# tprodanov/locityper

Hardware: AMD Instinct MI355X
Metric: reads/s through the whole genotyping path (scored + prefiltered + default solver scheme); reads_scored_per_s and genotypes_solved_per_s give the two halves (higher is better)
Workload: dtype f64

## Files before the change

### locityper_amd/csrc/lcty_api.hip

```cpp
#include <algorithm>
#include <cmath>
#include <memory>
#include <numeric>

#include "lcty_objects.hpp"

using namespace lcty;

namespace lcty {
static thread_local std::string g_last_error;
thread_local hipStream_t tl_stream = nullptr;
void set_last_error(const std::string& msg) { g_last_error = msg; }
}

hipEvent_t lcty_ctx::get_event() {
    hipEvent_t e;
    if (!event_pool.empty()) { e = event_pool.back(); event_pool.pop_back(); return e; }
    LCTY_HIP(hipEventCreate(&e));
    return e;
}

void lcty_ctx::fold_oldest(lcty::KernelTimer& t, size_t count) {
    count = std::min(count, t.pending.size());
    for (size_t i = 0; i < count; i++) {
        float ms = 0.f;
        LCTY_HIP(hipEventSynchronize(t.pending[i].second));
        LCTY_HIP(hipEventElapsedTime(&ms, t.pending[i].first, t.pending[i].second));
        t.total_ms += ms; t.launches++;
        event_pool.push_back(t.pending[i].first); event_pool.push_back(t.pending[i].second);
    }
    t.pending.erase(t.pending.begin(), t.pending.begin() + static_cast<std::ptrdiff_t>(count));
}

extern "C" {

int32_t lcty_ctx_set_knob(lcty_ctx* ctx, const char* name, int64_t value) {
    return guarded([&] {
        if (!ctx || !name) fail(LCTY_ERR_INVALID_INPUT, "null argument");
        static const char* const known[] = {"transfer_levels", "transfer_scratch_mb", "transfer_waves", "transfer_cap_new", "transfer_arena",
                                            "depth_table_start", "solve_budget_mb", "solve_chains_per_wave", "solve_extra_start", "solve_lds_weights",
                                            "anneal_lds_weights", "contig_info_slide", "gather_chunk_mb", "prefilter_gram", "prefilter_gram_cols",
                                            "prefilter_gram_levels", "comm_fail_at", "score_lean", "arena_cap_pct", "exact_threads", "host_threads",
                                            "score_lean_keep", "score_lean_two", "queue_early_head", "db_chunk_cols", "basis_batch_words",
                                            "align_batch_pairs", "align_hash_bits", "align_dp_cells", "align_match_budget", "align_cigar_store_mb", "pafvcf_hash_bits", "pafvcf_table_mb",
                                            "genome_max_bases", "sample_bam_hash_bits", "sample_bam_max_slice_bytes", "sample_bam_inflate",
                                            "bgzf_deflate", "bgzf_deflate_max_bytes", "aln_bam_max_slice_bytes", "vcf_max_slice_bytes",
#ifdef LCTY_DIAG
                                            "solve_stats", "queue_trace", "map_trace", "exact_trace", "solve_greedy_form", "solve_anneal_timing", "score_timing",
                                            "solve_init_tiles", "transfer_phases", "genome_scan_form",
#endif
                                            nullptr};
        bool ok = false;
        for (const char* const* k = known; *k; k++) ok |= strcmp(*k, name) == 0;
        if (!ok) fail(LCTY_ERR_INVALID_INPUT, "unknown knob '%s'", name);
        if (strcmp(name, "bgzf_deflate") == 0 && value != 0 && value != 1) fail(LCTY_ERR_INVALID_INPUT, "bgzf_deflate = %lld (0: host, 1: device)", static_cast<long long>(value));
        if (value < 0) ctx->knobs.erase(name); else ctx->knobs[name] = value;
    });
}

int32_t lcty_ctx_set_path(lcty_ctx* ctx, const char* name, const char* path) {
    return guarded([&] {
        if (!ctx || !name) fail(LCTY_ERR_INVALID_INPUT, "null argument");
        if (strcmp(name, "exact_dump") != 0) fail(LCTY_ERR_INVALID_INPUT, "unknown path '%s'", name);
        ctx->exact_dump_path = path ? path : "";
    });
}

const char* lcty_last_error(void) { return g_last_error.c_str(); }
const char* lcty_version(void) { return "locityper_hip 0.1.0 (gfx950)"; }

int32_t lcty_device_count(void) {
    int n = 0;
    if (hipGetDeviceCount(&n) != hipSuccess) { (void)hipGetLastError(); return 0; }
    return n;
}

int32_t lcty_ctx_create(int32_t device_id, lcty_ctx** out) {
    return guarded([&] {
        if (!out) fail(LCTY_ERR_INVALID_INPUT, "null argument");
        int n = 0;
        if (hipGetDeviceCount(&n) != hipSuccess || n == 0) {
            (void)hipGetLastError();
            fail(LCTY_ERR_RUNTIME, "no HIP device is visible: liblocityper_hip has no CPU fallback");
        }
        if (device_id < 0 || device_id >= n) fail(LCTY_ERR_INVALID_INPUT, "device %d out of range (0..%d)", device_id, n - 1);
        auto c = std::unique_ptr<lcty_ctx>(new lcty_ctx());
        c->device = device_id;
        LCTY_HIP(hipSetDevice(device_id));
        LCTY_HIP(hipGetDeviceProperties(&c->props, device_id));
        LCTY_HIP(hipStreamCreateWithFlags(&c->stream.main, hipStreamNonBlocking));
        *out = c.release();
    });
}
// ... 322 lines not shown
```

### locityper_amd/csrc/lcty_solve_device.hpp

```cpp
#pragma once
#include "lcty_objects.hpp"

namespace lcty {

constexpr uint32_t MAXP = 4;
constexpr uint32_t NONE32S = 0xFFFFFFFFu;
constexpr uint32_t MID_NONE24 = 0xFFFFFFu;
constexpr uint64_t WINDOW_KEY_XOR = 0xD1B54A32D192ED03ull;
constexpr uint64_t INIT_KEY_XOR = 0x8CB92BA72F3D8DD7ull;

struct FastDiv {
    uint32_t d, m, s1, s2;
    __host__ static FastDiv make(uint32_t d) {
        FastDiv f{d, 0, 0, 0};
        uint32_t l = 0;
        while ((1ull << l) < d) l++;
        f.m = static_cast<uint32_t>(((1ull << 32) * ((1ull << l) - d)) / d + 1);
        f.s1 = l < 1 ? l : 1; f.s2 = l > 0 ? l - 1 : 0;
        return f;
    }
    __device__ __forceinline__ uint32_t div(uint32_t n) const {
        const uint32_t t = __umulhi(m, n);
        return (t + ((n - t) >> s1)) >> s2;
    }
// ... 58 lines not shown
    uint32_t* c_uc;
    uint8_t* c_gc;
    uint32_t* c_depth;
    uint32_t* c_nnt;
    double* c_aln;
    double* liks;
    double* parts;
    uint32_t* overflow;
    double* dbg;
    uint32_t edge_trivial;
};

__device__ __forceinline__ uint64_t uniform64(uint64_t x) {
    const uint32_t lo = __builtin_amdgcn_readfirstlane(static_cast<uint32_t>(x));
    const uint32_t hi = __builtin_amdgcn_readfirstlane(static_cast<uint32_t>(x >> 32));
    return (static_cast<uint64_t>(hi) << 32) | lo;
}
__device__ __forceinline__ uint64_t counter_u64(uint64_t key, uint64_t i) {
    uint64_t z = key + (i + 1) * 0x9e3779b97f4a7c15ull;
    z = (z ^ (z >> 30)) * 0xbf58476d1ce4e5b9ull;
    z = (z ^ (z >> 27)) * 0x94d049bb133111ebull;
    return z ^ (z >> 31);
}
struct Xoshiro {
    uint64_t s0, s1, s2, s3;
    __device__ __forceinline__ void seed(uint64_t x) {
        s0 = counter_u64(x, 0); s1 = counter_u64(x, 1); s2 = counter_u64(x, 2); s3 = counter_u64(x, 3);
    }
    __device__ __forceinline__ uint64_t next() {
        const uint64_t sum = s0 + s3;
        const uint64_t result = ((sum << 23) | (sum >> 41)) + s0;
        const uint64_t t = s1 << 17;
        s2 ^= s0; s3 ^= s1; s1 ^= s2; s0 ^= s3; s2 ^= t; s3 = (s3 << 45) | (s3 >> 19);
        return result;
    }
    __device__ __forceinline__ uint64_t below(uint64_t n) { return __umul64hi(next(), n); }
    __device__ __forceinline__ double f64() { return static_cast<double>(next() >> 11) * (1.0 / 9007199254740992.0); }
};

constexpr uint32_t INIT_SEGS = 4;
struct RecList {
    ChainRec* base; const uint32_t* cum; uint32_t seg_reads;
    uint32_t r1 = 0, r2 = 0, r3 = 0; bool in_regs = false;
    __device__ __forceinline__ uint32_t place(uint32_t s) const {
        const uint32_t c1 = in_regs ? r1 : cum[1], c2 = in_regs ? r2 : cum[2], c3 = in_regs ? r3 : cum[3];
        const uint32_t k = (s >= c1 ? 1u : 0u) + (s >= c2 ? 1u : 0u) + (s >= c3 ? 1u : 0u);
        const uint32_t before = s >= c3 ? c3 : s >= c2 ? c2 : s >= c1 ? c1 : 0u;
        return s - before + k * seg_reads;
    }
    __device__ __forceinline__ ChainRec& operator[](uint32_t s) const { return base[place(s)]; }
};

constexpr uint32_t INIT_TILE_T = 8, INIT_TILE_R = 6;
constexpr uint32_t INIT_TILE_Q = 1024;
static_assert(INIT_TILE_Q >= 64 * (INIT_TILE_T + 1) && (INIT_TILE_Q & (INIT_TILE_Q - 1)) == 0, "the list holds a block's entries");
struct __attribute__((aligned(16))) InitChainP {
    uint64_t seed;
    uint32_t chain;
    uint32_t ia, ib;
    uint32_t row0, row1;
    uint32_t id0, id1;
    uint32_t shift0, rs0, re0, shift1, rs1, re1;
    uint32_t total_w;
};
static_assert(sizeof(InitChainP) == 64, "InitChainP layout");
struct __attribute__((aligned(16))) InitGroup { uint32_t first, n_chains, n_rows, _pad; uint32_t row[8]; };
static_assert(sizeof(InitGroup) == 48 && INIT_TILE_R <= 8, "InitGroup layout");
struct InitPlan {
    std::vector<InitGroup> groups; std::vector<InitChainP> chains;
    uint32_t T = 0, R = 0;
    size_t lds = 0;
};

inline void set_rec_list(SolveView& V, uint64_t n_reads) {
    V.seg_reads = static_cast<uint32_t>(((n_reads + INIT_SEGS - 1) / INIT_SEGS + 63) / 64 * 64);
    if (V.seg_reads == 0) V.seg_reads = 64;
    V.rstride = static_cast<uint64_t>(INIT_SEGS) * V.seg_reads;
}
inline size_t init_chain_lds(uint32_t wstride) { return ((static_cast<size_t>(wstride) * 4 + 15) & ~static_cast<size_t>(15)) + 256 * 8 + 64; }

template <typename... P, typename... A>
void launch_lds(lcty_ctx* ctx, int timer, void (*kernel)(P...), dim3 grid, dim3 block, size_t lds, hipStream_t s, const A&... args) {
    if (lds > 48 * 1024)
        LCTY_HIP(hipFuncSetAttribute(reinterpret_cast<const void*>(kernel), hipFuncAttributeMaxDynamicSharedMemorySize, static_cast<int>(lds)));
    auto go = [&] { hipLaunchKernelGGL(kernel, grid, block, lds, s, args...); };
    if (timer < 0) go();
    else ctx->timed(timer, go, s);
    LCTY_HIP(hipGetLastError());
}

void check_solver(const lcty_solver* solver);

void ensure_solver_tables(lcty_reads* reads);
void ensure_depth_table(lcty_locus* loc, uint64_t want);
void build_depth_table_into(const lcty_locus* loc, uint32_t depth, DevBuf<double>& out, hipStream_t s);
bool solver_lds_fits(uint32_t wstride);
struct InitHost {
    const uint16_t* genotypes; const uint64_t* seeds; const uint16_t* row_of; const lcty_locus* loc; uint32_t n_cus;
    uint32_t lds_budget;
};
void plan_init_groups(const SolveView& V, const InitHost& H, uint32_t nch, InitPlan& plan);
void launch_init(lcty_ctx* ctx, const SolveView& V, uint32_t nch, size_t lds_init, hipStream_t s, const InitHost* host, lcty_ctx::SolveWorkspace& ws,
                 InitPlan& plan);
void launch_greedy_chains(lcty_ctx* ctx, SolveView& V, uint32_t nch, hipStream_t stream, lcty_ctx::SolveWorkspace& ws);
void launch_anneal(lcty_ctx* ctx, const SolveView& V, uint32_t nch, hipStream_t s);
void launch_pause(hipStream_t s);
void launch_store_cur(ChainRec* recs, const uint32_t* words, uint64_t n, hipStream_t s);
void launch_pack_rows_count(uint64_t n, const LocCell* table, uint64_t ngp, uint32_t n_good, const uint16_t* alleles, uint32_t n_rows,
                            unsigned long long* total, hipStream_t s);
void launch_pack_rows(uint64_t n, const LocCell* table, const uint32_t* table_ext, const double* table_unm, uint64_t ngp, uint32_t n_good,
                      const uint16_t* alleles, uint32_t n_rows, const PairAlnDev* pa, LocEntry* cells, uint64_t out_stride, PairAlnDev* extras,
                      unsigned long long* cursor, hipStream_t s);
void launch_place_rows(uint64_t n, const LocEntry* cells, uint64_t in_stride, uint32_t n_good, uint32_t n_rows, uint32_t ext_base, LocCell* full,
                       uint32_t* full_ext, double* full_unm, bool write_unm, uint64_t full_stride, uint64_t first, hipStream_t s);
void launch_pad_rows(uint64_t n, LocCell* full, uint32_t* full_ext, double* full_unm, uint64_t full_stride, uint64_t from, uint32_t n_rows, hipStream_t s);
void launch_count_unexplained(uint32_t blocks, const uint8_t* status, const double* unmapped, const double* matrix, uint64_t n_pairs, uint32_t A,
                              const uint16_t* ids, uint32_t ploidy, unsigned long long* out, hipStream_t s);
void launch_read_nw(const SolveView& V, uint32_t* nw, hipStream_t s);
void launch_assignment_counts(const SolveView& V, const uint32_t* nw, const uint64_t* read_off, uint16_t* counts, hipStream_t s);

}
```

### locityper_amd/csrc/lcty_solve_kernels.hip

```cpp
#include <algorithm>
#include <cmath>
#include <type_traits>
#include <vector>

#include "lcty_solve_device.hpp"

namespace lcty {


__global__ __launch_bounds__(256) void build_loc_table_kernel(const uint32_t* __restrict__ good_ix, uint32_t n_good, uint64_t ngp,
                                                              uint32_t A, const uint32_t* __restrict__ pa_idx,
                                                              const uint64_t* __restrict__ pa_off, const PairAlnDev* __restrict__ pa,
                                                              const double* __restrict__ unmapped, LocCell* __restrict__ table,
                                                              uint32_t* __restrict__ table_ext, double* __restrict__ table_unm,
                                                              uint32_t* __restrict__ err) {
    __shared__ LocCell tile[32][33];
    __shared__ uint32_t tile_ext[32][33];
    const uint32_t g0 = blockIdx.x * 32, c0 = blockIdx.y * 32;
    const uint32_t tx = threadIdx.x & 31u, ty = threadIdx.x >> 5;
    if (blockIdx.y == 0 && threadIdx.x < 32) {
        const uint32_t g = g0 + threadIdx.x;
        if (g < ngp) table_unm[g] = g < n_good ? unmapped[good_ix[g]] : 0.0;
    }
    for (uint32_t i = ty; i < 32; i += 8) {
// ... 368 lines not shown
            LocIter<P> it; it.start(L);
            LocOut o;
            for (uint32_t t = 0; t < min(L.nw, 255u) && it.next(L, V, o); t++) {
                uint32_t wa, wb;
                loc_windows(V, G, o, seed, rp, t, &wa, &wb);
                const uint32_t win = wa | (wb << 16);
                if (t == 0) { rec.lp0 = o.lp; rec.win0 = win; }
                else if (t == 1) { rec.lp1 = o.lp; rec.win1 = win; }
                else if (room) { ExtraLoc e; e.lp = o.lp; e.win = win; e._pad = 0; extra[eix + t - 2] = e; }
                if (t == a0) {
                    atomicAdd(&depth[wa], 1u);
                    atomicAdd(&depth[wb], 1u);
                    aln_part += o.lp;
                }
            }
            if (nontrivial) recs[slot] = rec;
        }
    }
    if (lane == 0) seg_cnt[wave] = n_recs;
    red[tid] = aln_part;
    __syncthreads();
    const uint32_t ex_total = seg_cnt[4];
    if (tid == 0) {
        if (ex_total > V.extra_cap) { atomicMax(V.overflow, 4u); atomicMax(V.overflow + 1, ex_total); }
        if (ex_total >= (1u << 24)) atomicMax(V.overflow, 2u);
    }
    for (uint32_t s = 128; s > 0; s >>= 1) {
        if (tid < s) red[tid] += red[tid + s];
        __syncthreads();
    }
    uint32_t* gdepth = V.c_depth + static_cast<uint64_t>(chain) * V.wstride;
    for (uint32_t w = tid; w < G.total_w; w += 256) gdepth[w] = depth[w];
    if (tid == 0) {
        uint32_t* cum = V.c_seg + static_cast<uint64_t>(chain) * 4;
        uint32_t run = 0;
        for (uint32_t k = 0; k < INIT_SEGS; k++) { cum[k] = run; run += seg_cnt[k]; }
        V.c_aln[chain] = red[0]; V.c_nnt[chain] = run; V.c_totw[chain] = G.total_w;
    }
}

__device__ __forceinline__ uint64_t counter_fin(uint64_t z) {
    z = (z ^ (z >> 30)) * 0xbf58476d1ce4e5b9ull;
    z = (z ^ (z >> 27)) * 0x94d049bb133111ebull;
    return z ^ (z >> 31);
}
constexpr uint64_t GOLDEN64 = 0x9e3779b97f4a7c15ull;
typedef uint32_t u32x4_t __attribute__((ext_vector_type(4)));
__device__ __forceinline__ void store_16(uint4* p, uint4 v) {
    u32x4_t x; x.x = v.x; x.y = v.y; x.z = v.z; x.w = v.w;
    __builtin_nontemporal_store(x, reinterpret_cast<u32x4_t*>(p));
}
__host__ __device__ inline size_t init_tile_lds(uint32_t T, uint32_t R, uint32_t wstride) {
    const size_t depth = (static_cast<size_t>(T) * wstride * 4 + 15) & ~static_cast<size_t>(15);
    return depth + static_cast<size_t>(T) * 256 * 8 + 4ull * R * 64 * 16 + static_cast<size_t>(T) * 4 * 8 + static_cast<size_t>(T) * 4 * 5 + 64;
}

__device__ __forceinline__ void init_tile_deferred(const SolveView& V, const InitChainP* __restrict__ cp, uint32_t T, uint32_t* depth, double* aln_def,
                                                   uint32_t* ex_cnt, unsigned long long* queue, uint32_t head, uint32_t n, uint32_t wave, uint32_t lane, bool random_start) {
    double add = 0.0;
    uint32_t my_c = 0xFFFFFFFFu;
    if (lane < n) {
        const unsigned long long packed = __hip_atomic_load(&queue[(head + lane) & (INIT_TILE_Q - 1)], __ATOMIC_RELAXED, __HIP_MEMORY_SCOPE_WORKGROUP);
        const uint2 item = make_uint2(static_cast<uint32_t>(packed), static_cast<uint32_t>(packed >> 32));
        const uint32_t c = item.x >> 24, rp = item.x & 0xFFFFFFu, slot = item.y;
        const InitChainP P = cp[c];
        Geno<2> G;
        G.id[0] = P.id0; G.id[1] = P.id1; G.row[0] = P.row0; G.row[1] = P.row1; G.shift[0] = P.shift0; G.shift[1] = P.shift1;
        G.reg_start[0] = P.rs0; G.reg_start[1] = P.rs1; G.reg_end[0] = P.re0; G.reg_end[1] = P.re1; G.total_w = P.total_w;
        Locs<2> L;
        locs_init<2>(L, V, rp, G);
        if (L.nw > 255) atomicMax(V.overflow, 2u);
        uint32_t a0 = 0;
        if (L.nw > 1 && random_start)
            a0 = static_cast<uint32_t>(__umul64hi(counter_u64(P.seed ^ INIT_KEY_XOR, rp), static_cast<uint64_t>(L.nw)));
        const uint32_t nloc = min(L.nw, 255u), n_extra = nloc > 2 ? nloc - 2u : 0u;
        uint32_t eix = 0;
        if (n_extra) eix = atomicAdd(&ex_cnt[c], n_extra);
        const bool room = static_cast<uint64_t>(eix) + n_extra <= V.extra_cap;
        ExtraLoc* extra = V.extra + static_cast<uint64_t>(P.chain) * V.extra_cap;
        ChainRec rec; rec.rp_cur = rp | (a0 << 24); rec.meta = nloc | (eix << 8);
        rec.lp0 = rec.lp1 = 0.0; rec.win0 = rec.win1 = 0;
        LocIter<2> it; it.start(L);
        LocOut o;
        for (uint32_t t = 0; t < nloc && it.next(L, V, o); t++) {
            uint32_t wa, wb;
            loc_windows(V, G, o, P.seed, rp, t, &wa, &wb);
            const uint32_t win = wa | (wb << 16);
            if (t == 0) { rec.lp0 = o.lp; rec.win0 = win; }
            else if (t == 1) { rec.lp1 = o.lp; rec.win1 = win; }
            else if (room) { ExtraLoc e; e.lp = o.lp; e.win = win; e._pad = 0; extra[eix + t - 2] = e; }
            if (t == a0) {
                atomicAdd(&depth[static_cast<size_t>(c) * V.wstride + wa], 1u);
                atomicAdd(&depth[static_cast<size_t>(c) * V.wstride + wb], 1u);
                add = o.lp;
                my_c = c;
            }
        }
        if (L.nw > 1) V.recs[static_cast<uint64_t>(P.chain) * V.rstride + static_cast<uint64_t>(wave) * V.seg_reads + slot] = rec;
    }
    for (uint32_t c = 0; c < T; c++) {
        unsigned long long m = __ballot(my_c == c);
        if (!m) continue;
        double acc = aln_def[c * 4 + wave];
        while (m) {
            const int l = __ffsll(static_cast<long long>(m)) - 1;
            acc += __hiloint2double(__builtin_amdgcn_readlane(__double2hiint(add), l), __builtin_amdgcn_readlane(__double2loint(add), l));
            m &= m - 1;
        }
        if (lane == 0) aln_def[c * 4 + wave] = acc;
    }
}

__global__ __launch_bounds__(256) void solve_init_tile_kernel(const SolveView V, const InitGroup* __restrict__ groups, const InitChainP* __restrict__ chains,
                                                             unsigned long long* lists, const uint32_t T_max, const uint32_t R_max) {
    extern __shared__ __align__(16) uint8_t smem[];
    const uint32_t tid = threadIdx.x, lane = tid & 63u, wave = __builtin_amdgcn_readfirstlane(tid >> 6);
    const InitGroup& grp = groups[blockIdx.x];
    const uint32_t T = grp.n_chains, R = grp.n_rows;
    const InitChainP* __restrict__ cp = chains + grp.first;
    const uint32_t W = V.wstride;
    uint32_t* depth = reinterpret_cast<uint32_t*>(smem);
    size_t at = (static_cast<size_t>(T_max) * W * 4 + 15) & ~static_cast<size_t>(15);
    double* aln = reinterpret_cast<double*>(smem + at); at += static_cast<size_t>(T_max) * 256 * 8;
    uint4* stage = reinterpret_cast<uint4*>(smem + at) + static_cast<size_t>(wave) * R_max * 64; at += 4ull * R_max * 64 * 16;
    unsigned long long* queue = lists + (static_cast<size_t>(blockIdx.x) * 4 + wave) * INIT_TILE_Q;
    double* aln_def = reinterpret_cast<double*>(smem + at); at += static_cast<size_t>(T_max) * 4 * 8;
    uint32_t* ex_cnt = reinterpret_cast<uint32_t*>(smem + at); at += static_cast<size_t>(T_max) * 4;
    uint32_t* seg_cnt = reinterpret_cast<uint32_t*>(smem + at);

    for (uint32_t c = 0; c < T; c++) {
        const InitChainP P = cp[c];
        double* ww = V.c_ww + static_cast<uint64_t>(P.chain) * W;
        uint8_t* wgc = V.c_gc + static_cast<uint64_t>(P.chain) * W;
        uint32_t* wuc = V.n_wk ? V.c_uc + static_cast<uint64_t>(P.chain) * W : nullptr;
        for (uint32_t w = tid; w < P.total_w; w += 256) {
            depth[c * W + w] = 0;
            double weight = 0.0; uint32_t g = 0, uc = V.n_wk - 1;
            if (w >= 2) {
                const bool second = w >= P.shift1;
                const uint32_t allele = second ? P.id1 : P.id0, sh = second ? P.shift1 : P.shift0, rs = second ? P.rs1 : P.rs0;
                const uint32_t start = rs + (w - sh) * V.window, end = start + V.window;
                const uint32_t left = min(V.tweak, start), right = min(V.tweak, V.allele_len[allele] - end);
                const uint64_t r = counter_u64(P.seed ^ WINDOW_KEY_XOR, w);
                const int64_t off = -static_cast<int64_t>(left) + static_cast<int64_t>(__umul64hi(r, static_cast<uint64_t>(left + right + 1)));
                const uint32_t wstart = static_cast<uint32_t>(static_cast<int64_t>(start) + off);
                const uint32_t i = V.ci_off[allele] + (wstart > V.left_padding ? wstart - V.left_padding : 0u);
                weight = V.win_weight[i];
                g = V.gc[i];
                if (wuc) uc = V.uniq_cnt[i] | (static_cast<uint32_t>(V.compl_cnt[i]) << 16);
                if (weight < V.min_weight || weight < 1e-7) { weight = 0.0; g = 0; uc = V.n_wk - 1; }
            }
            ww[w] = weight; wgc[w] = static_cast<uint8_t>(g);
            if (wuc) wuc[w] = uc;
        }
        aln[c * 256 + tid] = 0.0;
        if (tid < 4) aln_def[c * 4 + tid] = 0.0;
        if (tid == 0) ex_cnt[c] = 0;
    }
    __syncthreads();

    const bool random_start = V.solver.kind == LCTY_SOLVER_ANNEAL || (V.solver.kind == LCTY_SOLVER_GREEDY && !V.solver.best_start);
    const uint32_t seg_lo = min(wave * V.seg_reads, V.n_good), seg_hi = min(seg_lo + V.seg_reads, V.n_good);
    uint64_t row_at[INIT_TILE_R];
#pragma unroll
    for (uint32_t r = 0; r < INIT_TILE_R; r++) row_at[r] = static_cast<uint64_t>(grp.row[r < R ? r : 0]) * V.ngp;
    const uint4* __restrict__ table = reinterpret_cast<const uint4*>(V.table);
    uint4 nxt[INIT_TILE_R]; double nxt_unm = 0.0;
#pragma unroll
    for (uint32_t r = 0; r < INIT_TILE_R; r++) nxt[r] = make_uint4(0, 0, 0, 0);
    if (seg_lo + lane < seg_hi) {
#pragma unroll
        for (uint32_t r = 0; r < INIT_TILE_R; r++) if (r < R) nxt[r] = table[row_at[r] + seg_lo + lane];
        nxt_unm = V.table_unm[seg_lo + lane];
    }
    uint32_t n_recs_all = 0;
    uint32_t qn = 0, qhead = 0;
    for (uint32_t base = seg_lo; base < seg_hi; base += 64) {
        const uint32_t rp = base + lane;
        const bool in = rp < seg_hi;
#pragma unroll
        for (uint32_t r = 0; r < INIT_TILE_R; r++) if (r < R) stage[r * 64 + lane] = nxt[r];
        const double unm = nxt_unm;
        if (rp + 64 < seg_hi) {
#pragma unroll
            for (uint32_t r = 0; r < INIT_TILE_R; r++) if (r < R) nxt[r] = table[row_at[r] + rp + 64];
            nxt_unm = V.table_unm[rp + 64];
        }
        const uint64_t zbase = ((static_cast<uint64_t>(rp) << 16) + 1ull) * GOLDEN64;
        const uint64_t abase = (static_cast<uint64_t>(rp) + 1ull) * GOLDEN64;
        for (uint32_t c = 0; c < T; c++) {
            const InitChainP P = cp[c];
            const uint4 qa = stage[P.ia * 64 + lane], qb = stage[P.ib * 64 + lane];
            const double aln_before = aln[c * 256 + tid];
            const double lpA = __hiloint2double(static_cast<int>(qa.y), static_cast<int>(qa.x));
            const double lpB = __hiloint2double(static_cast<int>(qb.y), static_cast<int>(qb.x));
            const uint32_t rawA = qa.z >> 24, rawB = qb.z >> 24;
            const double thresh = fmax(fmax(lpA, lpB), unm) - V.prob_diff;
            const bool kA = in && rawA != 0 && lpA >= thresh, kB = in && rawB != 0 && lpB >= thresh, kU = in && unm >= thresh;
            const bool multi = (kA && rawA > 1) || (kB && rawB > 1);
            const uint32_t nw = (kA ? 1u : 0u) + (kB ? 1u : 0u) + (kU ? 1u : 0u);
            bool nontrivial = nw > 1;
            if (__any(multi && nw == 1)) {
                if (multi && nw == 1) {
                    const uint32_t ext = V.table_ext[static_cast<uint64_t>(kA ? P.row0 : P.row1) * V.ngp + rp];
                    nontrivial = V.pa[ext].ln_prob >= thresh;
                }
            }
            const unsigned long long nt_mask = __ballot(nontrivial);
            const uint32_t before = __builtin_amdgcn_readlane(n_recs_all, c);
            const uint32_t slot = before + static_cast<uint32_t>(__popcll(nt_mask & ((1ull << lane) - 1ull)));
            {
                const uint32_t after = __builtin_amdgcn_readfirstlane(before + static_cast<uint32_t>(__popcll(nt_mask)));
                uint32_t m0_was;
                asm volatile("s_mov_b32 %1, m0\n\ts_mov_b32 m0, %3\n\tv_writelane_b32 %0, %2, m0\n\ts_mov_b32 m0, %1"
                             : "+v"(n_recs_all), "=&s"(m0_was) : "s"(after), "s"(c));
            }
            const unsigned long long mm = __ballot(multi);
            if (mm) {
                if (multi)
                    __hip_atomic_store(&queue[(qhead + qn + static_cast<uint32_t>(__popcll(mm & ((1ull << lane) - 1ull)))) & (INIT_TILE_Q - 1)],
                                       static_cast<unsigned long long>(rp | (c << 24)) | (static_cast<unsigned long long>(slot) << 32), __ATOMIC_RELAXED,
                                       __HIP_MEMORY_SCOPE_WAVEFRONT);
                qn += static_cast<uint32_t>(__popcll(mm));
            }
            const bool BgtA = lpB > lpA, UgtA = unm > lpA, UgtB = unm > lpB;
            const uint32_t posA = ((kB && BgtA) ? 1u : 0u) + ((kU && UgtA) ? 1u : 0u);
            const uint32_t posB = ((kA && !BgtA) ? 1u : 0u) + ((kU && UgtB) ? 1u : 0u);
            uint32_t tA1 = 0, tA2 = 0, tB1 = 0, tB2 = 0;
            if (V.tweak) {
                const uint64_t z0 = P.seed + zbase;
                const uint64_t rA = counter_fin(z0 + (posA == 0 ? 0ull : posA == 1 ? GOLDEN64 : 2ull * GOLDEN64));
                const uint64_t rB = counter_fin(z0 + (posB == 0 ? 0ull : posB == 1 ? GOLDEN64 : 2ull * GOLDEN64));
                tA1 = V.by_tweak.mod(static_cast<uint32_t>(rA >> 32)); tA2 = V.by_tweak.mod(static_cast<uint32_t>(rA));
                tB1 = V.by_tweak.mod(static_cast<uint32_t>(rB >> 32)); tB2 = V.by_tweak.mod(static_cast<uint32_t>(rB));
            }
            auto window_ix = [&](uint32_t mid, bool none, uint32_t tw, uint32_t rs, uint32_t re, uint32_t sh) -> uint32_t {
                const uint32_t m = mid + tw;
                uint32_t q = V.by_window.div(m - rs) + sh;
                asm volatile("" : "+v"(q));
                const uint32_t inside = (rs <= m && m < re) ? q : 1u;
                return none ? 0u : inside;
            };
            const uint32_t midA1 = qa.z & MID_NONE24, midB1 = qb.z & MID_NONE24;
            const uint32_t winA = window_ix(midA1, midA1 == MID_NONE24, tA1, P.rs0, P.re0, P.shift0) |
                                  (window_ix(qa.w, qa.w == NONE32S, tA2, P.rs0, P.re0, P.shift0) << 16);
            const uint32_t winB = window_ix(midB1, midB1 == MID_NONE24, tB1, P.rs1, P.re1, P.shift1) |
                                  (window_ix(qb.w, qb.w == NONE32S, tB2, P.rs1, P.re1, P.shift1) << 16);
            const bool a_0 = kA && posA == 0, b_0 = kB && posB == 0, a_1 = kA && posA == 1, b_1 = kB && posB == 1, a_2 = kA && posA == 2, b_2 = kB && posB == 2;
            const double lp0 = a_0 ? lpA : (b_0 ? lpB : unm), lp1 = a_1 ? lpA : (b_1 ? lpB : unm), lp2 = a_2 ? lpA : (b_2 ? lpB : unm);
            const uint32_t win0 = a_0 ? winA : (b_0 ? winB : 0u), win1 = a_1 ? winA : (b_1 ? winB : 0u), win2 = a_2 ? winA : (b_2 ? winB : 0u);
            uint32_t a0 = 0;
            double lps = lp0; uint32_t wins = win0;
            if (random_start) {
                const uint64_t r = counter_fin((P.seed ^ INIT_KEY_XOR) + abase);
                a0 = nw > 1 ? static_cast<uint32_t>(__umul64hi(r, static_cast<uint64_t>(nw))) : 0u;
                lps = a0 == 0 ? lp0 : (a0 == 1 ? lp1 : lp2); wins = a0 == 0 ? win0 : (a0 == 1 ? win1 : win2);
            }
            const bool fast = !multi && nw != 0;
            if (fast) {
                atomicAdd(&depth[c * W + (wins & 0xFFFFu)], 1u);
                atomicAdd(&depth[c * W + (wins >> 16)], 1u);
                aln[c * 256 + tid] = aln_before + lps;
            }
            uint32_t eix = 0;
            if (fast && nw == 3) {
                eix = atomicAdd(&ex_cnt[c], 1u);
                if (eix < V.extra_cap) {
                    ExtraLoc e; e.lp = lp2; e.win = win2; e._pad = 0;
                    V.extra[static_cast<uint64_t>(P.chain) * V.extra_cap + eix] = e;
                }
            }
            if (fast && nw > 1) {
                uint4* dst = reinterpret_cast<uint4*>(V.recs + static_cast<uint64_t>(P.chain) * V.rstride + static_cast<uint64_t>(wave) * V.seg_reads + slot);
                store_16(dst, make_uint4(rp | (a0 << 24), nw | (eix << 8), static_cast<uint32_t>(__double2loint(lp0)), static_cast<uint32_t>(__double2hiint(lp0))));
                store_16(dst + 1, make_uint4(static_cast<uint32_t>(__double2loint(lp1)), static_cast<uint32_t>(__double2hiint(lp1)), win0, win1));
            }
        }
        const bool last = base + 64 >= seg_hi;
        if (qn >= 64 || (last && qn)) {
            __builtin_amdgcn_fence(__ATOMIC_RELEASE, "workgroup");
            __builtin_amdgcn_wave_barrier();
            __builtin_amdgcn_fence(__ATOMIC_ACQUIRE, "workgroup");
            while (qn >= 64 || (last && qn)) {
                const uint32_t n = min(qn, 64u);
                init_tile_deferred(V, cp, T, depth, aln_def, ex_cnt, queue, qhead, n, wave, lane, random_start);
                qhead = (qhead + n) & (INIT_TILE_Q - 1); qn -= n;
            }
        }
    }
    if (lane < T) seg_cnt[lane * 4 + wave] = n_recs_all;
    __syncthreads();
    for (uint32_t c = 0; c < T; c++) {
        const InitChainP P = cp[c];
        const uint32_t ex_total = ex_cnt[c];
        if (tid == 0) {
            if (ex_total > V.extra_cap) { atomicMax(V.overflow, 4u); atomicMax(V.overflow + 1, ex_total); }
            if (ex_total >= (1u << 24)) atomicMax(V.overflow, 2u);
        }
        uint32_t* gdepth = V.c_depth + static_cast<uint64_t>(P.chain) * W;
        for (uint32_t w = tid; w < P.total_w; w += 256) gdepth[w] = depth[c * W + w];
        if (wave == 0) {
            double v = (aln[c * 256 + lane] + aln[c * 256 + 64 + lane]) + (aln[c * 256 + 128 + lane] + aln[c * 256 + 192 + lane]);
            for (int o = 32; o > 0; o >>= 1) v += __shfl_xor(v, o);
            v += (aln_def[c * 4] + aln_def[c * 4 + 1]) + (aln_def[c * 4 + 2] + aln_def[c * 4 + 3]);
            if (lane == 0) {
                uint32_t* cum = V.c_seg + static_cast<uint64_t>(P.chain) * 4;
                uint32_t run = 0;
                for (uint32_t k = 0; k < INIT_SEGS; k++) { cum[k] = run; run += seg_cnt[c * 4 + k]; }
                V.c_aln[P.chain] = v; V.c_nnt[P.chain] = run; V.c_totw[P.chain] = P.total_w;
            }
        }
    }
}

struct PairGather { int32_t c[2]; uint32_t dmax[2]; double weight[2], vnew[2], vold[2]; };
__device__ __forceinline__ double pair_term(const PairGather& g, int i, uint32_t* deepest) {
    const bool live = g.c[i] != 0 && g.weight[i] != 0.0;
    *deepest = max(*deepest, live ? g.dmax[i] : 0u);
    return live ? g.weight[i] * g.vnew[i] - g.weight[i] * g.vold[i] : 0.0;
}

__device__ __forceinline__ double lut_at(const double* lut, uint32_t index) {
    return *reinterpret_cast<const double*>(reinterpret_cast<const char*>(lut) + (index << 3));
}
constexpr uint32_t DEPTH_MASK = 0x1FFFFFFu;
struct WinGathered {
    static constexpr bool WEIGHTS_LAST = false;
    uint32_t* wd;
    const double* ww;
    struct Word { uint32_t word; };
    __device__ __forceinline__ Word at(uint32_t w) const { return Word{wd[w]}; }
    __device__ __forceinline__ uint32_t depth(Word x) const { return x.word & DEPTH_MASK; }
    __device__ __forceinline__ uint32_t gc(Word x) const { return x.word >> 25; }
    __device__ __forceinline__ double weight(Word x, uint32_t w) const { return ww[w]; }
};
constexpr uint32_t LW_DEPTH_BITS = 23, LW_DEPTH_MASK = (1u << LW_DEPTH_BITS) - 1u;
struct WinTables {
    static constexpr bool WEIGHTS_LAST = true;
    uint32_t* wd;
    const uint16_t* wh;
    const double* wk; const double* wc;
    struct Word { uint32_t word, half; };
    __device__ __forceinline__ Word at(uint32_t w) const { return Word{wd[w], wh[w]}; }
    __device__ __forceinline__ uint32_t depth(Word x) const { return x.word & LW_DEPTH_MASK; }
    __device__ __forceinline__ uint32_t gc(Word x) const { return x.half & 0x7Fu; }
    __device__ __forceinline__ double weight(Word x, uint32_t w) const { return wk[x.word >> LW_DEPTH_BITS] * wc[x.half >> 7]; }
};

template <typename LAYOUT>
struct Chain {
    const SolveView* V;
    LAYOUT L;
    using Word = typename LAYOUT::Word;
    __device__ __forceinline__ double wlp_at(uint32_t w) const {
        const Word x = L.at(w);
// ... 1041 lines not shown
    int64_t mode = ctx->knob("anneal_lds_weights", tables ? 2 : 0);
    if (mode == 2 && !tables) mode = 0;
    if (mode == 2) launch_anneal_as<2>(ctx, V, nch, s);
    else if (mode == 1) launch_anneal_as<1>(ctx, V, nch, s);
    else launch_anneal_as<0>(ctx, V, nch, s);
}

void launch_greedy_chains(lcty_ctx* ctx, SolveView& V, uint32_t nch, hipStream_t stream, lcty_ctx::SolveWorkspace& ws) {
    const uint32_t S = V.solver.sample_size;
    const uint64_t simds = 4ull * static_cast<uint64_t>(ctx->props.multiProcessorCount);
    uint32_t lpc = S <= 16 ? 16 : S <= 32 ? 32 : 64;
    if (lpc == 16 && (nch + 3) / 4 > simds) {
        if (S <= 12 && (nch + 4) / 5 <= simds) lpc = 12;
        else if (S <= 10) lpc = 10;
        else if (S <= 12) lpc = 12;
    }
    const int64_t want = ctx->knob("solve_chains_per_wave", 0);
    if (want > 0) {
        const uint32_t forced = want >= 6 ? 10u : want == 5 ? 12u : static_cast<uint32_t>(64 / std::min<int64_t>(want, 4));
        if (forced >= S) lpc = forced;
    }
    const bool lw = V.n_wk != 0 && 2 * static_cast<uint64_t>(V.n_good) + 2 <= LW_DEPTH_MASK && ctx->knob("solve_lds_weights", 1) != 0;
    while (lpc < 64 && greedy_lds(lpc, V, lw) > 80 * 1024) lpc = lpc < 16 ? 16 : lpc * 2;
    auto go = [&](auto tag) {
        constexpr uint32_t L = decltype(tag)::value;
        if (lw) launch_greedy<L, true>(ctx, V, nch, stream); else launch_greedy<L, false>(ctx, V, nch, stream);
    };
    const bool timed_form = lpc == 12 && lw && (ctx->diag_knob("solve_greedy_form", 0) & 32) != 0;
    const size_t n_waves = (static_cast<size_t>(nch) + 4) / 5 + 2;
    V.dbg = nullptr;
    if (timed_form) { ws.dbg.ensure(12 * n_waves); ws.dbg.zero(stream); V.dbg = ws.dbg.p; }
    if (lpc == 10) go(std::integral_constant<uint32_t, 10>{});
    else if (lpc == 12) go(std::integral_constant<uint32_t, 12>{});
    else if (lpc == 16) go(std::integral_constant<uint32_t, 16>{});
    else if (lpc == 32) go(std::integral_constant<uint32_t, 32>{});
    else go(std::integral_constant<uint32_t, 64>{});
    if (timed_form) {
        std::vector<double> d(12 * n_waves);
        ws.dbg.download(d.data(), d.size(), stream);
        LCTY_HIP(hipStreamSynchronize(stream));
        double sum[12] = {0}; size_t used = 0;
        for (size_t w = 0; w < n_waves; w++) if (d[12 * w + 6] > 0) { used++; for (int k = 0; k < 12; k++) sum[k] += d[12 * w + k] / d[12 * w + 6]; }
        if (used) fprintf(stderr, "[lcty greedy phases] %zu wavefronts; clock ticks per iteration: candidates+requests %.0f (waiting for the further locations %.0f, current location %.0f, its pair %.0f, first alternative %.0f), ext+sample+record request %.0f, wait+score %.0f, row best %.0f, move %.0f; loop total %.0f; a round for the second alternative in %.3f of the iterations\n",
                          used, sum[0] / used, sum[11] / used, sum[8] / used, sum[9] / used, sum[10] / used, sum[1] / used, sum[2] / used, sum[3] / used, sum[4] / used, sum[5] / used, sum[7] / used);
    }
}

bool solver_lds_fits(uint32_t wstride) {
    return !(static_cast<size_t>(wstride) * 12 + sizeof(AnnealRing) + 128 > 160 * 1024 || wstride > 65535);
}
void plan_init_groups(const SolveView& V, const InitHost& H, uint32_t nch, InitPlan& plan) {
    plan.groups.clear(); plan.chains.clear(); plan.T = plan.R = 0; plan.lds = 0;
    const uint32_t attempts = V.attempts, ng = (nch + attempts - 1) / attempts, A = V.A;
    uint32_t T_cap = INIT_TILE_T;
    const size_t lds_budget = H.lds_budget ? H.lds_budget : 80 * 1024;
    while (T_cap > 1 && init_tile_lds(T_cap, std::min(INIT_TILE_R, T_cap + 1), V.wstride) > lds_budget) T_cap--;
    const uint64_t per_cu = std::max<uint64_t>(1, std::min<uint64_t>(160 * 1024 / init_tile_lds(T_cap, std::min(INIT_TILE_R, T_cap + 1), V.wstride), 4));
    const uint64_t places = per_cu * std::max(1u, H.n_cus);
    T_cap = static_cast<uint32_t>(std::max<uint64_t>(1, std::min<uint64_t>(T_cap, (nch + places - 1) / places)));
    const uint32_t R_cap = std::min(INIT_TILE_R, T_cap + 1);
    std::vector<uint32_t> deg(A, 0), rank(A, 0), order(A);
    for (uint32_t g = 0; g < ng; g++) { deg[H.genotypes[2 * g]]++; deg[H.genotypes[2 * g + 1]]++; }
    for (uint32_t a = 0; a < A; a++) order[a] = a;
    std::stable_sort(order.begin(), order.end(), [&](uint32_t x, uint32_t y) { return deg[x] > deg[y]; });
    for (uint32_t r = 0; r < A; r++) rank[order[r]] = r;
    std::vector<uint32_t> gts(ng);
    std::vector<uint64_t> key(ng);
    for (uint32_t g = 0; g < ng; g++) {
        const uint32_t ra = rank[H.genotypes[2 * g]], rb = rank[H.genotypes[2 * g + 1]];
        const uint64_t u = std::min(ra, rb), v = std::max(ra, rb);
        key[g] = ((u / 2) << 48) | ((v / 4) << 32) | (u << 16) | v;
        gts[g] = g;
    }
    std::sort(gts.begin(), gts.end(), [&](uint32_t x, uint32_t y) { return key[x] != key[y] ? key[x] < key[y] : x < y; });
    auto row_of = [&](uint32_t allele) -> uint32_t { return H.row_of ? H.row_of[allele] : allele; };
    struct Unit { uint32_t gi, a0, n; };
    struct Proto { std::vector<Unit> units; uint32_t n_chains = 0, n_rows = 0; uint32_t row[8] = {0, 0, 0, 0, 0, 0, 0, 0}; };
    std::vector<Proto> protos;
    Proto cur;
    auto close = [&] { if (cur.n_chains) protos.push_back(cur); cur = Proto{}; };
    auto fresh_rows = [&](const Proto& p, uint32_t r0, uint32_t r1) -> uint32_t {
        bool h0 = false, h1 = false;
        for (uint32_t r = 0; r < p.n_rows; r++) { h0 |= p.row[r] == r0; h1 |= p.row[r] == r1; }
        return (h0 ? 0u : 1u) + ((h1 || r1 == r0) ? 0u : 1u);
    };
    auto add_rows = [&](Proto& p, uint32_t r0, uint32_t r1) {
        for (uint32_t x : {r0, r1}) {
            bool have = false;
            for (uint32_t r = 0; r < p.n_rows; r++) have |= p.row[r] == x;
            if (!have) p.row[p.n_rows++] = x;
        }
    };
    for (uint32_t gi : gts) {
        const uint32_t r0 = row_of(H.genotypes[2 * gi]), r1 = row_of(H.genotypes[2 * gi + 1]);
        for (uint32_t a0 = 0; a0 < attempts;) {
            const uint32_t want = std::min(attempts - a0, T_cap);
            if (cur.n_chains + want > T_cap || cur.n_rows + fresh_rows(cur, r0, r1) > R_cap) close();
            add_rows(cur, r0, r1);
            cur.units.push_back(Unit{gi, a0, want}); cur.n_chains += want;
            a0 += want;
        }
    }
    close();
    std::stable_sort(protos.begin(), protos.end(), [](const Proto& a, const Proto& b) { return a.n_chains > b.n_chains; });
    if (protos.size() > places) {
        uint64_t tail_chains = 0;
        for (size_t i = places; i < protos.size(); i++) tail_chains += protos[i].n_chains;
        const uint32_t piece = static_cast<uint32_t>(std::max<uint64_t>(1, std::min<uint64_t>(T_cap, tail_chains / (3 * places))));
        std::vector<Proto> tail;
        for (size_t i = places; i < protos.size(); i++) {
            Proto part;
            for (const Unit& u : protos[i].units)
                for (uint32_t done = 0; done < u.n;) {
                    const uint32_t take = std::min(u.n - done, piece - part.n_chains);
                    add_rows(part, row_of(H.genotypes[2 * u.gi]), row_of(H.genotypes[2 * u.gi + 1]));
                    part.units.push_back(Unit{u.gi, u.a0 + done, take}); part.n_chains += take;
                    done += take;
                    if (part.n_chains == piece) { tail.push_back(part); part = Proto{}; }
                }
            if (part.n_chains) tail.push_back(part);
        }
        protos.resize(places);
        protos.insert(protos.end(), tail.begin(), tail.end());
    }
    for (const Proto& p : protos) {
        InitGroup g{};
        g.first = static_cast<uint32_t>(plan.chains.size()); g.n_rows = p.n_rows;
        for (uint32_t r = 0; r < 8; r++) g.row[r] = p.row[r];
        for (const Unit& u : p.units) {
            const uint32_t id0 = H.genotypes[2 * u.gi], id1 = H.genotypes[2 * u.gi + 1];
            const uint32_t row0 = row_of(id0), row1 = row_of(id1);
            uint32_t ia = 0, ib = 0;
            for (uint32_t r = 0; r < p.n_rows; r++) { if (p.row[r] == row0) ia = r; if (p.row[r] == row1) ib = r; }
            const uint32_t nw0 = H.loc->n_windows[id0], nw1 = H.loc->n_windows[id1];
            for (uint32_t k = 0; k < u.n; k++) {
                const uint32_t chain = u.gi * attempts + u.a0 + k;
                if (chain >= nch) break;
                InitChainP P{};
                P.seed = H.seeds[chain]; P.chain = chain; P.ia = ia; P.ib = ib; P.row0 = row0; P.row1 = row1; P.id0 = id0; P.id1 = id1;
                P.shift0 = 2; P.rs0 = H.loc->reg_start[id0]; P.re0 = P.rs0 + nw0 * V.window;
                P.shift1 = 2 + nw0; P.rs1 = H.loc->reg_start[id1]; P.re1 = P.rs1 + nw1 * V.window;
                P.total_w = 2 + nw0 + nw1;
                plan.chains.push_back(P);
                g.n_chains++;
            }
        }
        if (!g.n_chains) continue;
        plan.T = std::max(plan.T, g.n_chains); plan.R = std::max(plan.R, g.n_rows);
        plan.groups.push_back(g);
    }
    plan.lds = init_tile_lds(plan.T, plan.R, V.wstride);
}

void launch_init(lcty_ctx* ctx, const SolveView& V, uint32_t nch, size_t lds_init, hipStream_t s, const InitHost* host, lcty_ctx::SolveWorkspace& ws,
                 InitPlan& plan) {
    if (V.ploidy == 2 && host && nch && ctx->diag_knob("solve_init_tiles", 1) != 0) {
        plan_init_groups(V, *host, nch, plan);
        const size_t gb = plan.groups.size() * sizeof(InitGroup), cb = plan.chains.size() * sizeof(InitChainP);
        if (ctx->diag_knob("solve_stats", 0)) {
            uint64_t rows = 0; uint32_t hist[INIT_TILE_T + 1] = {0};
            for (const InitGroup& g : plan.groups) { rows += g.n_rows; hist[g.n_chains]++; }
            fprintf(stderr, "[lcty solve] initialisation: %u chains in %zu groups (largest %u chains, %u rows; %.2f rows per chain; LDS %zu B); groups of 1..%u chains:",
                    nch, plan.groups.size(), plan.T, plan.R, static_cast<double>(rows) / nch, plan.lds, INIT_TILE_T);
            for (uint32_t t = 1; t <= INIT_TILE_T; t++) fprintf(stderr, " %u", hist[t]);
            fprintf(stderr, "\n");
        }
        const size_t lb = plan.groups.size() * 4 * INIT_TILE_Q * sizeof(unsigned long long);
        ws.init_plan.ensure_slack(gb + cb + lb);
        LCTY_HIP(hipMemcpyAsync(ws.init_plan.p, plan.groups.data(), gb, hipMemcpyHostToDevice, s));
        LCTY_HIP(hipMemcpyAsync(ws.init_plan.p + gb, plan.chains.data(), cb, hipMemcpyHostToDevice, s));
        launch_lds(ctx, V.solver.kind == LCTY_SOLVER_ANNEAL ? LCTY_K_SOLVE_INIT_ANNEAL : LCTY_K_SOLVE_INIT, solve_init_tile_kernel,
                   dim3(static_cast<uint32_t>(plan.groups.size())), dim3(256), plan.lds, s, V, reinterpret_cast<const InitGroup*>(ws.init_plan.p),
                   reinterpret_cast<const InitChainP*>(ws.init_plan.p + gb), reinterpret_cast<unsigned long long*>(ws.init_plan.p + gb + cb), plan.T, plan.R);
        return;
    }
    switch (V.ploidy) {
        case 1: launch_init_p<1>(ctx, V, nch, lds_init, s); break;
        case 2: launch_init_p<2>(ctx, V, nch, lds_init, s); break;
        case 3: launch_init_p<3>(ctx, V, nch, lds_init, s); break;
        default: launch_init_p<4>(ctx, V, nch, lds_init, s); break;
    }
}
void launch_pause(hipStream_t s) { hipLaunchKernelGGL(pause_kernel, dim3(1), dim3(64), 0, s, 8u); }
void launch_store_cur(ChainRec* recs, const uint32_t* words, uint64_t n, hipStream_t s) {
    hipLaunchKernelGGL(store_cur_kernel, dim3(static_cast<uint32_t>((n + 255) / 256)), dim3(256), 0, s, recs, words, n);
    LCTY_HIP(hipGetLastError());
}
void launch_pack_rows_count(uint64_t n, const LocCell* table, uint64_t ngp, uint32_t n_good, const uint16_t* alleles, uint32_t n_rows,
                            unsigned long long* total, hipStream_t s) {
    hipLaunchKernelGGL(pack_rows_count_kernel, dim3(static_cast<uint32_t>((n + 255) / 256)), dim3(256), 0, s, table, ngp, n_good, alleles, n_rows, total);
    LCTY_HIP(hipGetLastError());
}
void launch_pack_rows(uint64_t n, const LocCell* table, const uint32_t* table_ext, const double* table_unm, uint64_t ngp, uint32_t n_good,
                      const uint16_t* alleles, uint32_t n_rows, const PairAlnDev* pa, LocEntry* cells, uint64_t out_stride, PairAlnDev* extras,
                      unsigned long long* cursor, hipStream_t s) {
    hipLaunchKernelGGL(pack_rows_kernel, dim3(static_cast<uint32_t>((n + 255) / 256)), dim3(256), 0, s, table, table_ext, table_unm, ngp, n_good, alleles,
                       n_rows, pa, cells, out_stride, extras, cursor);
    LCTY_HIP(hipGetLastError());
}
void launch_place_rows(uint64_t n, const LocEntry* cells, uint64_t in_stride, uint32_t n_good, uint32_t n_rows, uint32_t ext_base, LocCell* full,
                       uint32_t* full_ext, double* full_unm, bool write_unm, uint64_t full_stride, uint64_t first, hipStream_t s) {
    hipLaunchKernelGGL(place_rows_kernel, dim3(static_cast<uint32_t>((n + 255) / 256)), dim3(256), 0, s, cells, in_stride, n_good, n_rows, ext_base, full,
                       full_ext, full_unm, write_unm, full_stride, first);
    LCTY_HIP(hipGetLastError());
}
void launch_pad_rows(uint64_t n, LocCell* full, uint32_t* full_ext, double* full_unm, uint64_t full_stride, uint64_t from, uint32_t n_rows, hipStream_t s) {
    hipLaunchKernelGGL(pad_rows_kernel, dim3(static_cast<uint32_t>((n + 255) / 256)), dim3(256), 0, s, full, full_ext, full_unm, full_stride, from, n_rows);
    LCTY_HIP(hipGetLastError());
}
void launch_count_unexplained(uint32_t blocks, const uint8_t* status, const double* unmapped, const double* matrix, uint64_t n_pairs, uint32_t A,
// ... 23 lines not shown
```

Measured before the change: 2.724 million.

## Keep per-chain alignment sums in registers and reshape init tile grouping

```diff
diff --git a/locityper_amd/csrc/lcty_api.hip b/locityper_amd/csrc/lcty_api.hip
--- a/locityper_amd/csrc/lcty_api.hip
+++ b/locityper_amd/csrc/lcty_api.hip
@@ -39,6 +39,7 @@
         if (!ctx || !name) fail(LCTY_ERR_INVALID_INPUT, "null argument");
         static const char* const known[] = {"transfer_levels", "transfer_scratch_mb", "transfer_waves", "transfer_cap_new", "transfer_arena",
                                             "depth_table_start", "solve_budget_mb", "solve_chains_per_wave", "solve_extra_start", "solve_lds_weights",
+                                            "solve_init_chains", "solve_init_rows", "solve_init_places",
                                             "anneal_lds_weights", "contig_info_slide", "gather_chunk_mb", "prefilter_gram", "prefilter_gram_cols",
                                             "prefilter_gram_levels", "comm_fail_at", "score_lean", "arena_cap_pct", "exact_threads", "host_threads",
                                             "score_lean_keep", "score_lean_two", "queue_early_head", "db_chunk_cols", "basis_batch_words",
diff --git a/locityper_amd/csrc/lcty_solve_device.hpp b/locityper_amd/csrc/lcty_solve_device.hpp
--- a/locityper_amd/csrc/lcty_solve_device.hpp
+++ b/locityper_amd/csrc/lcty_solve_device.hpp
@@ -134,6 +134,7 @@
 };
 
 constexpr uint32_t INIT_TILE_T = 8, INIT_TILE_R = 6;
+constexpr uint32_t INIT_TILE_T_DEFAULT = 6, INIT_TILE_R_DEFAULT = 5;
 constexpr uint32_t INIT_TILE_Q = 1024;
 static_assert(INIT_TILE_Q >= 64 * (INIT_TILE_T + 1) && (INIT_TILE_Q & (INIT_TILE_Q - 1)) == 0, "the list holds a block's entries");
 struct __attribute__((aligned(16))) InitChainP {
@@ -180,6 +181,8 @@
 struct InitHost {
     const uint16_t* genotypes; const uint64_t* seeds; const uint16_t* row_of; const lcty_locus* loc; uint32_t n_cus;
     uint32_t lds_budget;
+    uint32_t max_chains = 0, max_rows = 0;
+    uint32_t places = 0;
 };
 void plan_init_groups(const SolveView& V, const InitHost& H, uint32_t nch, InitPlan& plan);
 void launch_init(lcty_ctx* ctx, const SolveView& V, uint32_t nch, size_t lds_init, hipStream_t s, const InitHost* host, lcty_ctx::SolveWorkspace& ws,
diff --git a/locityper_amd/csrc/lcty_solve_kernels.hip b/locityper_amd/csrc/lcty_solve_kernels.hip
--- a/locityper_amd/csrc/lcty_solve_kernels.hip
+++ b/locityper_amd/csrc/lcty_solve_kernels.hip
@@ -444,7 +444,7 @@
 }
 __host__ __device__ inline size_t init_tile_lds(uint32_t T, uint32_t R, uint32_t wstride) {
     const size_t depth = (static_cast<size_t>(T) * wstride * 4 + 15) & ~static_cast<size_t>(15);
-    return depth + static_cast<size_t>(T) * 256 * 8 + 4ull * R * 64 * 16 + static_cast<size_t>(T) * 4 * 8 + static_cast<size_t>(T) * 4 * 5 + 64;
+    return depth + 2ull * 256 * 8 + 4ull * R * 64 * 16 + static_cast<size_t>(T) * 4 * 8 + static_cast<size_t>(T) * 4 * 5 + 64;
 }
 
 __device__ __forceinline__ void init_tile_deferred(const SolveView& V, const InitChainP* __restrict__ cp, uint32_t T, uint32_t* depth, double* aln_def,
@@ -513,7 +513,7 @@
     const uint32_t W = V.wstride;
     uint32_t* depth = reinterpret_cast<uint32_t*>(smem);
     size_t at = (static_cast<size_t>(T_max) * W * 4 + 15) & ~static_cast<size_t>(15);
-    double* aln = reinterpret_cast<double*>(smem + at); at += static_cast<size_t>(T_max) * 256 * 8;
+    double* red = reinterpret_cast<double*>(smem + at); at += 2ull * 256 * 8;
     uint4* stage = reinterpret_cast<uint4*>(smem + at) + static_cast<size_t>(wave) * R_max * 64; at += 4ull * R_max * 64 * 16;
     unsigned long long* queue = lists + (static_cast<size_t>(blockIdx.x) * 4 + wave) * INIT_TILE_Q;
     double* aln_def = reinterpret_cast<double*>(smem + at); at += static_cast<size_t>(T_max) * 4 * 8;
@@ -545,7 +545,6 @@
             ww[w] = weight; wgc[w] = static_cast<uint8_t>(g);
             if (wuc) wuc[w] = uc;
         }
-        aln[c * 256 + tid] = 0.0;
         if (tid < 4) aln_def[c * 4 + tid] = 0.0;
         if (tid == 0) ex_cnt[c] = 0;
     }
@@ -567,6 +566,9 @@
     }
     uint32_t n_recs_all = 0;
     uint32_t qn = 0, qhead = 0;
+    double acc[INIT_TILE_T];
+#pragma unroll
+    for (uint32_t c = 0; c < INIT_TILE_T; c++) acc[c] = 0.0;
     for (uint32_t base = seg_lo; base < seg_hi; base += 64) {
         const uint32_t rp = base + lane;
         const bool in = rp < seg_hi;
@@ -580,10 +582,10 @@
         }
         const uint64_t zbase = ((static_cast<uint64_t>(rp) << 16) + 1ull) * GOLDEN64;
         const uint64_t abase = (static_cast<uint64_t>(rp) + 1ull) * GOLDEN64;
-        for (uint32_t c = 0; c < T; c++) {
+#pragma unroll
+        for (uint32_t c = 0; c < INIT_TILE_T; c++) if (c < T) {
             const InitChainP P = cp[c];
             const uint4 qa = stage[P.ia * 64 + lane], qb = stage[P.ib * 64 + lane];
-            const double aln_before = aln[c * 256 + tid];
             const double lpA = __hiloint2double(static_cast<int>(qa.y), static_cast<int>(qa.x));
             const double lpB = __hiloint2double(static_cast<int>(qb.y), static_cast<int>(qb.x));
             const uint32_t rawA = qa.z >> 24, rawB = qb.z >> 24;
@@ -638,29 +640,33 @@
                                   (window_ix(qa.w, qa.w == NONE32S, tA2, P.rs0, P.re0, P.shift0) << 16);
             const uint32_t winB = window_ix(midB1, midB1 == MID_NONE24, tB1, P.rs1, P.re1, P.shift1) |
                                   (window_ix(qb.w, qb.w == NONE32S, tB2, P.rs1, P.re1, P.shift1) << 16);
-            const bool a_0 = kA && posA == 0, b_0 = kB && posB == 0, a_1 = kA && posA == 1, b_1 = kB && posB == 1, a_2 = kA && posA == 2, b_2 = kB && posB == 2;
-            const double lp0 = a_0 ? lpA : (b_0 ? lpB : unm), lp1 = a_1 ? lpA : (b_1 ? lpB : unm), lp2 = a_2 ? lpA : (b_2 ? lpB : unm);
-            const uint32_t win0 = a_0 ? winA : (b_0 ? winB : 0u), win1 = a_1 ? winA : (b_1 ? winB : 0u), win2 = a_2 ? winA : (b_2 ? winB : 0u);
+            const bool a_0 = kA && posA == 0, b_0 = kB && posB == 0, a_1 = kA && posA == 1, b_1 = kB && posB == 1;
+            const double lp0 = a_0 ? lpA : (b_0 ? lpB : unm), lp1 = a_1 ? lpA : (b_1 ? lpB : unm);
+            const uint32_t win0 = a_0 ? winA : (b_0 ? winB : 0u), win1 = a_1 ? winA : (b_1 ? winB : 0u);
             uint32_t a0 = 0;
             double lps = lp0; uint32_t wins = win0;
             if (random_start) {
                 const uint64_t r = counter_fin((P.seed ^ INIT_KEY_XOR) + abase);
                 a0 = nw > 1 ? static_cast<uint32_t>(__umul64hi(r, static_cast<uint64_t>(nw))) : 0u;
-                lps = a0 == 0 ? lp0 : (a0 == 1 ? lp1 : lp2); wins = a0 == 0 ? win0 : (a0 == 1 ? win1 : win2);
+                lps = a0 == 0 ? lp0 : lp1; wins = a0 == 0 ? win0 : win1;
             }
             const bool fast = !multi && nw != 0;
-            if (fast) {
-                atomicAdd(&depth[c * W + (wins & 0xFFFFu)], 1u);
-                atomicAdd(&depth[c * W + (wins >> 16)], 1u);
-                aln[c * 256 + tid] = aln_before + lps;
-            }
             uint32_t eix = 0;
             if (fast && nw == 3) {
+                const bool a_2 = posA == 2, b_2 = posB == 2;
+                const double lp2 = a_2 ? lpA : (b_2 ? lpB : unm);
+                const uint32_t win2 = a_2 ? winA : (b_2 ? winB : 0u);
+                if (a0 == 2) { lps = lp2; wins = win2; }
                 eix = atomicAdd(&ex_cnt[c], 1u);
                 if (eix < V.extra_cap) {
                     ExtraLoc e; e.lp = lp2; e.win = win2; e._pad = 0;
                     V.extra[static_cast<uint64_t>(P.chain) * V.extra_cap + eix] = e;
                 }
+            }
+            if (fast) {
+                atomicAdd(&depth[c * W + (wins & 0xFFFFu)], 1u);
+                atomicAdd(&depth[c * W + (wins >> 16)], 1u);
+                acc[c] += lps;
             }
             if (fast && nw > 1) {
                 uint4* dst = reinterpret_cast<uint4*>(V.recs + static_cast<uint64_t>(P.chain) * V.rstride + static_cast<uint64_t>(wave) * V.seg_reads + slot);
@@ -682,7 +688,8 @@
     }
     if (lane < T) seg_cnt[lane * 4 + wave] = n_recs_all;
     __syncthreads();
-    for (uint32_t c = 0; c < T; c++) {
+#pragma unroll
+    for (uint32_t c = 0; c < INIT_TILE_T; c++) if (c < T) {
         const InitChainP P = cp[c];
         const uint32_t ex_total = ex_cnt[c];
         if (tid == 0) {
@@ -691,8 +698,11 @@
         }
         uint32_t* gdepth = V.c_depth + static_cast<uint64_t>(P.chain) * W;
         for (uint32_t w = tid; w < P.total_w; w += 256) gdepth[w] = depth[c * W + w];
+        double* aln = red + (c & 1u) * 256;
+        aln[tid] = acc[c];
+        __syncthreads();
         if (wave == 0) {
-            double v = (aln[c * 256 + lane] + aln[c * 256 + 64 + lane]) + (aln[c * 256 + 128 + lane] + aln[c * 256 + 192 + lane]);
+            double v = (aln[lane] + aln[64 + lane]) + (aln[128 + lane] + aln[192 + lane]);
             for (int o = 32; o > 0; o >>= 1) v += __shfl_xor(v, o);
             v += (aln_def[c * 4] + aln_def[c * 4 + 1]) + (aln_def[c * 4 + 2] + aln_def[c * 4 + 3]);
             if (lane == 0) {
@@ -1840,13 +1850,15 @@
 void plan_init_groups(const SolveView& V, const InitHost& H, uint32_t nch, InitPlan& plan) {
     plan.groups.clear(); plan.chains.clear(); plan.T = plan.R = 0; plan.lds = 0;
     const uint32_t attempts = V.attempts, ng = (nch + attempts - 1) / attempts, A = V.A;
-    uint32_t T_cap = INIT_TILE_T;
+    const uint32_t T_lim = H.max_chains ? std::min(H.max_chains, INIT_TILE_T) : INIT_TILE_T_DEFAULT;
+    const uint32_t R_lim = H.max_rows ? std::min(std::max(H.max_rows, 2u), INIT_TILE_R) : INIT_TILE_R_DEFAULT;
+    uint32_t T_cap = T_lim;
     const size_t lds_budget = H.lds_budget ? H.lds_budget : 80 * 1024;
-    while (T_cap > 1 && init_tile_lds(T_cap, std::min(INIT_TILE_R, T_cap + 1), V.wstride) > lds_budget) T_cap--;
-    const uint64_t per_cu = std::max<uint64_t>(1, std::min<uint64_t>(160 * 1024 / init_tile_lds(T_cap, std::min(INIT_TILE_R, T_cap + 1), V.wstride), 4));
-    const uint64_t places = per_cu * std::max(1u, H.n_cus);
+    while (T_cap > 1 && init_tile_lds(T_cap, std::min(R_lim, T_cap + 1), V.wstride) > lds_budget) T_cap--;
+    const uint64_t per_cu = std::max<uint64_t>(1, std::min<uint64_t>(160 * 1024 / init_tile_lds(T_cap, std::min(R_lim, T_cap + 1), V.wstride), 4));
+    const uint64_t places = H.places ? H.places : per_cu * std::max(1u, H.n_cus);
     T_cap = static_cast<uint32_t>(std::max<uint64_t>(1, std::min<uint64_t>(T_cap, (nch + places - 1) / places)));
-    const uint32_t R_cap = std::min(INIT_TILE_R, T_cap + 1);
+    const uint32_t R_cap = std::min(R_lim, T_cap + 1);
     std::vector<uint32_t> deg(A, 0), rank(A, 0), order(A);
     for (uint32_t g = 0; g < ng; g++) { deg[H.genotypes[2 * g]]++; deg[H.genotypes[2 * g + 1]]++; }
     for (uint32_t a = 0; a < A; a++) order[a] = a;
@@ -1854,10 +1866,11 @@
     for (uint32_t r = 0; r < A; r++) rank[order[r]] = r;
     std::vector<uint32_t> gts(ng);
     std::vector<uint64_t> key(ng);
+    const uint64_t tile_v = std::max(1u, T_cap / 2);
     for (uint32_t g = 0; g < ng; g++) {
         const uint32_t ra = rank[H.genotypes[2 * g]], rb = rank[H.genotypes[2 * g + 1]];
         const uint64_t u = std::min(ra, rb), v = std::max(ra, rb);
-        key[g] = ((u / 2) << 48) | ((v / 4) << 32) | (u << 16) | v;
+        key[g] = ((u / 2) << 48) | ((v / tile_v) << 32) | (u << 16) | v;
         gts[g] = g;
     }
     std::sort(gts.begin(), gts.end(), [&](uint32_t x, uint32_t y) { return key[x] != key[y] ? key[x] < key[y] : x < y; });
@@ -1943,7 +1956,11 @@
 void launch_init(lcty_ctx* ctx, const SolveView& V, uint32_t nch, size_t lds_init, hipStream_t s, const InitHost* host, lcty_ctx::SolveWorkspace& ws,
                  InitPlan& plan) {
     if (V.ploidy == 2 && host && nch && ctx->diag_knob("solve_init_tiles", 1) != 0) {
-        plan_init_groups(V, *host, nch, plan);
+        InitHost shaped = *host;
+        shaped.max_chains = static_cast<uint32_t>(std::max<int64_t>(0, ctx->knob("solve_init_chains", 0)));
+        shaped.max_rows = static_cast<uint32_t>(std::max<int64_t>(0, ctx->knob("solve_init_rows", 0)));
+        shaped.places = static_cast<uint32_t>(std::max<int64_t>(0, ctx->knob("solve_init_places", 0)));
+        plan_init_groups(V, shaped, nch, plan);
         const size_t gb = plan.groups.size() * sizeof(InitGroup), cb = plan.chains.size() * sizeof(InitChainP);
         if (ctx->diag_knob("solve_stats", 0)) {
             uint64_t rows = 0; uint32_t hist[INIT_TILE_T + 1] = {0};
```

Result: slower. 2.654 million (-2.6%).
